# wangheda/youtube-8m

Measured on AMD Instinct MI355X. Metric: training videos/sec, higher is better.
Workload: dtype f32; 1 GPU; BASELINE configs[3]: LstmModel (2 x BasicLSTMCell(1024), dynamic_rnn over F=300) on raw uint8 [B,300,1152] frames + MoeModel head (2 mixtures, V=4716), fp32 training step (fwd+bwd+clip+Adam); per_gpu_batch=128, global_batch=128, frames=300, parallelism=dp1, params=113902808

## Files before the change

include/yt8m_hip.h:

```cpp
#ifndef YT8M_HIP_H
#define YT8M_HIP_H
#include <stdint.h>

#ifdef __cplusplus
extern "C" {
#endif

typedef void* yt8m_stream_t;

enum yt8m_status { YT8M_OK = 0, YT8M_E_BADARG = -1, YT8M_E_SHAPE = -2, YT8M_E_HIP = -3, YT8M_E_RCCL = -4 };
enum yt8m_label_dtype { YT8M_LABEL_U8 = 0, YT8M_LABEL_F32 = 1 };

int yt8m_abi_version(void);
const char* yt8m_last_error(void);
const char* yt8m_built_arch(void);

int yt8m_prof_enable(int on);
int yt8m_prof_reset(void);
int yt8m_prof_get(int family, int64_t* launches, double* total_ms);
int yt8m_prof_get_flops(int family, double* flops);
int yt8m_prof_get_bytes(int family, double* bytes);

int yt8m_probe_mfma_f32(int iters, int blocks, float* sink, yt8m_stream_t stream);
int yt8m_probe_mfma_bf16(int iters, int blocks, int random_operands, float* sink, yt8m_stream_t stream);
int yt8m_probe_copy_f32(const float* src, float* dst, int64_t n, yt8m_stream_t stream);
int yt8m_probe_placement(int* out, int blocks, int spin_ticks, yt8m_stream_t stream);
int yt8m_stream_create_cu_mask(const uint32_t* mask, int words, yt8m_stream_t* stream);
int yt8m_stream_destroy(yt8m_stream_t stream);

int yt8m_gemm_f32(int transA, int transB, int64_t M, int64_t N, int64_t K,
                  const float* A, int64_t lda, const float* B, int64_t ldb,
                  float* C, int64_t ldc, const float* bias, float beta, yt8m_stream_t stream);

int yt8m_gemm_f32_batched(int transA, int transB, int64_t M, int64_t N, int64_t K,
                          const float* A, int64_t lda, int64_t strideA, const float* B, int64_t ldb, int64_t strideB,
                          float* C, int64_t ldc, int64_t strideC, float beta, int64_t batch, yt8m_stream_t stream);

typedef struct yt8m_gemm_problem {
  int64_t M, N, K;
  const void* A; int64_t lda;
  const void* B; int64_t ldb;
  float* C; int64_t ldc;
  const float* bias;
  float beta;
} yt8m_gemm_problem;
int64_t yt8m_gemm_workspace_bytes(void);
int yt8m_gemm_f32_grouped(int transA, int transB, int nprob, const yt8m_gemm_problem* probs, void* workspace,
                          int64_t workspace_bytes, yt8m_stream_t stream);
int yt8m_gemm_bf16_nt_grouped(int nprob, const yt8m_gemm_problem* probs, void* workspace, int64_t workspace_bytes,
                              yt8m_stream_t stream);
int64_t yt8m_x3_image_bytes(int64_t rows, int64_t K);
int yt8m_x3_split(const float* src, int64_t R, int64_t C, int64_t ld, float scale, void* plain, void* trans, yt8m_stream_t stream);
int yt8m_gemm_x3_nt_grouped(int nprob, const yt8m_gemm_problem* probs, void* workspace, int64_t workspace_bytes,
                            yt8m_stream_t stream);
int yt8m_h2_split(const float* src, int64_t R, int64_t C, int64_t ld, float scale, const float* dscale, void* plain, void* trans,
                  float* colpart, yt8m_stream_t stream);
int yt8m_h2_absmax(const float* src, int64_t R, int64_t C, int64_t ld, void* word, yt8m_stream_t stream);
int yt8m_h2_degraded(uint64_t* counts, int reset, yt8m_stream_t stream);
int yt8m_h2_split_dropout(const float* src, int64_t R, int64_t C, float scale, const float* dscale, void* plain, void* trans,
                          float keep_prob, uint64_t seed, int64_t offset, yt8m_stream_t stream);
int yt8m_h2_split_rowmax(const float* src, int64_t R, int64_t C, int64_t ld, const void* rowmax, float* inv, void* plain,
                         yt8m_stream_t stream);
int yt8m_h2_split_ex(const float* src, int64_t R, int64_t C, int64_t ld, float scale, const void* dscale, const float* rowscale, void* plain,
                     void* trans, void* trans_scaled, float* colpart, float* colpart_scaled, yt8m_stream_t stream);
int yt8m_gemm_h1x2_nt_ex(int64_t M, int64_t N, int64_t K, const void* A1, int64_t ska, const void* B2, int64_t skb, float* C, int64_t ldc,
                         const float* bias, float alpha, const void* dsb, const float* rowscale, const float* colsum, float colsum_scale,
                         float beta, void* workspace, int64_t workspace_bytes, yt8m_stream_t stream);
int yt8m_h2_rowscales(const float* src, int64_t R, int64_t C, int64_t ld, float* S, float* inv, yt8m_stream_t stream);
int yt8m_h2_split_rows(const float* src, int64_t R, int64_t C, int64_t ld, const float* S, void* plain, yt8m_stream_t stream);
int yt8m_gemm_h2_nt_ex(int64_t M, int64_t N, int64_t K, const void* A2, int64_t ska, const void* B2, int64_t skb, float* C, int64_t ldc,
                       const float* bias, float alpha, const void* dsa, const void* dsb, const float* rowscale, float beta, void* workspace,
                       int64_t workspace_bytes, yt8m_stream_t stream);
int yt8m_timepool_max_f32(const float* y, int64_t F, int64_t B, int64_t N, int64_t ldy, float* out, int32_t* idx, int64_t ldo,
                          yt8m_stream_t stream);
int yt8m_timepool_shiftmax_f32(const float* z, int64_t F, int64_t B, int64_t ldz, int nfilt, const int32_t* fs, const int32_t* ncol, float* out,
                               int32_t* idx, int64_t ldo, yt8m_stream_t stream);
int yt8m_u8_cnn_pool_dw(const uint8_t* q, const float* r_tm, const int32_t* idx, const float* g, int64_t ldg, int64_t B, int64_t F, int64_t D,
                        int64_t N, int64_t fs, float* dW, float beta, yt8m_stream_t stream);
int yt8m_f32_cnn_pool_dw(const float* x, int64_t ldx, const int32_t* idx, const float* g, int64_t ldg, int64_t B, int64_t F, int64_t D,
                         int64_t N, int64_t fs, float* dW, int64_t lddw, float beta, yt8m_stream_t stream);
int yt8m_f32_cnn_pool_dx(const int32_t* idx, const float* g, int64_t ldg, int64_t B, int64_t F, int64_t D, int nfilt, const float* const* wt,
                         const int32_t* fs, const int32_t* ncol, float* dx, int64_t lddx, yt8m_stream_t stream);
int yt8m_u8_frames_image_f16(const uint8_t* q, const int32_t* num_frames, int64_t B, int64_t F, int64_t D, float eps, void* image,
                             float* x_tm, float* r_out, yt8m_stream_t stream);
int yt8m_u8_frames_image_t_f16(const uint8_t* q, const int32_t* num_frames, int64_t B, int64_t F, int64_t D, void* image_t,
                               yt8m_stream_t stream);
int yt8m_gemm_h2_nt_grouped(int nprob, const yt8m_gemm_problem* probs, const float* alphas, const float* const* dsa,
                            const float* const* dsb, void* workspace, int64_t workspace_bytes, yt8m_stream_t stream);
int yt8m_x3_set_combine(int mode);
int yt8m_x3_set_schedule(int mode);
#define YT8M_GEMM_ROLE_DW 0x100
#define YT8M_GEMM_ROLE_H2 0x200
int yt8m_gemm_x3_pays(int64_t M, int64_t N, int64_t K);
int64_t yt8m_gemm_auto_scratch_bytes(int transA, int transB, int nprob, const yt8m_gemm_problem* probs);
int yt8m_gemm_auto_grouped(int transA, int transB, int nprob, const yt8m_gemm_problem* probs, void* workspace,
                           int64_t workspace_bytes, void* image_scratch, int64_t image_scratch_bytes, uint64_t* used_x3,
                           yt8m_stream_t stream);
int yt8m_gemm_auto_grouped_ex(int transA, int transB, int nprob, const yt8m_gemm_problem* probs, const float* const* absmaxA,
                              const float* const* absmaxB, void* workspace, int64_t workspace_bytes, void* image_scratch,
                              int64_t image_scratch_bytes, uint64_t* used_x3, yt8m_stream_t stream);
int yt8m_gemm_x1x3_nt(int64_t M, int64_t N, int64_t K, const void* A1, const void* B3, float* C, int64_t ldc, const float* bias,
                      const float* rowscale, const float* colsum, float colsum_scale, void* workspace, int64_t workspace_bytes,
                      yt8m_stream_t stream);
int yt8m_gemm_x1x3_nt_ex(int64_t M, int64_t N, int64_t K, const void* A1, int64_t ska, const void* B3, int64_t skb, float* C,
                         int64_t ldc, const float* bias, float alpha, const float* rowscale, const float* colsum,
                         float colsum_scale, float beta, void* workspace, int64_t workspace_bytes, yt8m_stream_t stream);
int yt8m_bf16_image(const float* src, int64_t R, int64_t C, int64_t ld, float scale, void* plain, void* trans, yt8m_stream_t stream);
int yt8m_gemm_b1_nt_grouped(int nprob, const yt8m_gemm_problem* probs, void* workspace, int64_t workspace_bytes, yt8m_stream_t stream);
int yt8m_gemm_b1_nt_grouped_bf16c(int nprob, const yt8m_gemm_problem* probs, unsigned c_bf16_mask, void* workspace, int64_t workspace_bytes,
                                  yt8m_stream_t stream);
int yt8m_moe_mix_fwd_bf16z(const void* Zg, const void* Ze, float* p, int64_t B, int64_t V, int M, yt8m_stream_t stream);
int yt8m_moe_mix_bwd_bf16_images_z16(const void* Zg, const void* Ze, const float* dp, const void* labels, int label_dtype, int64_t B,
                                     int64_t V, int M, float eps, float dscale, const float* upstream_dev, void* dZg_img, int64_t g_kb,
                                     void* dZg_t_img, int64_t gt_kb, void* dZe_img, int64_t e_kb, void* dZe_t_img, int64_t et_kb,
                                     float* be_part, yt8m_stream_t stream);
int yt8m_bf16_image_colsum(const float* src, int64_t R, int64_t C, int64_t ld, float scale, const float* rowscale, void* plain,
                           void* trans, void* trans_scaled, float* colpart, float* colpart_scaled, yt8m_stream_t stream);
int yt8m_gemm_b1_nt_ex(int64_t M, int64_t N, int64_t K, const void* A1, int64_t ska, const void* B1, int64_t skb, float* C, int64_t ldc,
                       const float* bias, float alpha, const float* rowscale, const float* colsum, float colsum_scale, float beta,
                       void* workspace, int64_t workspace_bytes, yt8m_stream_t stream);
int yt8m_x3_split_ex(const float* src, int64_t R, int64_t C, int64_t ld, float scale, const float* rowscale, void* plain,
                     void* trans, void* trans_scaled, yt8m_stream_t stream);
int yt8m_x3_split_colsum(const float* src, int64_t R, int64_t C, int64_t ld, float scale, const float* rowscale, void* plain,
                         void* trans, void* trans_scaled, float* colpart, float* colpart_scaled, yt8m_stream_t stream);
int yt8m_cast_f32_bf16(const float* src, int64_t rows, int64_t cols, int64_t ld, void* dst, int64_t dst_ld, int transpose,
                       yt8m_stream_t stream);
int yt8m_cast_f32_bf16_dual(const float* src, int64_t rows, int64_t cols, int64_t ld, void* dst_plain, int64_t plain_ld,
                            void* dst_trans, int64_t trans_ld, yt8m_stream_t stream);

int yt8m_l2norm_fwd_f32(const float* x, float* y, int64_t rows, int64_t cols, float eps, yt8m_stream_t stream);
int yt8m_l2norm_bwd_f32(const float* x, const float* dy, float* dx, int64_t rows, int64_t cols, float eps,
                        yt8m_stream_t stream);
int yt8m_dequant_l2norm_u8(const uint8_t* q, const int32_t* num_frames, float* x,
                           int64_t B, int64_t F, int64_t D, float eps, yt8m_stream_t stream);
int yt8m_dequant_mean_l2norm_u8(const uint8_t* q, const int32_t* num_frames, float* x,
                                int64_t B, int64_t F, int64_t D, float eps, yt8m_stream_t stream);
int yt8m_resolution_mean_u8(const uint8_t* q, const int32_t* num_frames, float* y, int32_t* num_frames_out, int64_t B, int64_t F,
                            int64_t D, int64_t resolution, int l2norm, float eps, yt8m_stream_t stream);
int yt8m_resolution_mean_f32(const float* x, const int32_t* num_frames, float* y, int32_t* num_frames_out, int64_t B, int64_t F,
                             int64_t D, int64_t resolution, int l2norm, float eps, yt8m_stream_t stream);
int yt8m_frame_pyramid_u8(const uint8_t* q, const int32_t* num_frames, int64_t B, int64_t F, int64_t D, int levels, int nseg,
// ... 586 lines not shown
```

youtube-8m_amd/_lib.py:

```python
import ctypes
import os

_HERE = os.path.dirname(os.path.abspath(__file__))
LIB_PATH = os.environ.get("YT8M_LIB", os.path.join(_HERE, "libyt8m_hip.so"))

c_void_p, c_int, c_int64, c_float, c_double = ctypes.c_void_p, ctypes.c_int, ctypes.c_int64, ctypes.c_float, ctypes.c_double
P = c_void_p

class GemmProblem(ctypes.Structure):
    _fields_ = [("M", c_int64), ("N", c_int64), ("K", c_int64), ("A", c_void_p), ("lda", c_int64), ("B", c_void_p),
                ("ldb", c_int64), ("C", c_void_p), ("ldc", c_int64), ("bias", c_void_p), ("beta", c_float)]


STREAM_HOOK = ctypes.CFUNCTYPE(None, ctypes.c_void_p, ctypes.c_void_p)


class PersistBwdImages(ctypes.Structure):
    _fields_ = [("plain", ctypes.c_void_p), ("trans", ctypes.c_void_p), ("trans_scaled", ctypes.c_void_p), ("rowscale", ctypes.c_void_p),
                ("colpart", ctypes.c_void_p), ("colpart_scaled", ctypes.c_void_p)]


class LstmStackDesc(ctypes.Structure):
    _fields_ = [("B", c_int64), ("F", c_int64), ("D", c_int64), ("H", c_int64), ("L", ctypes.c_int32), ("input_u8", ctypes.c_int32),
                ("forget_bias", c_float), ("fwd_chunks", ctypes.c_int32), ("bwd_chunks", ctypes.c_int32), ("need_dx", ctypes.c_int32),
# ... 196 lines not shown
    "yt8m_lstm_persist_fwd_bf16": (c_int, [P, P, c_int64, P, P, P, P, c_int64, c_int64, c_int64, c_int64, c_float, P, c_int64, P]),
    "yt8m_lstm_persist_bwd_supported": (c_int, [c_int64, c_int64]),
    "yt8m_lstm_persist_bwd": (c_int, [P, P, c_int64, P, P, P, P, c_int, P, P, c_int64, c_int64, c_int64, c_int64, P, c_int64, P]),
    "yt8m_lstm_persist_bwd_bf16": (c_int, [P, P, c_int64, P, P, P, P, c_int, P, P, c_int64, c_int64, c_int64, c_int64, P, c_int64, P]),
    "yt8m_lstm_persist_fwd_h2": (c_int, [P, P, c_int64, P, P, P, P, c_int64, c_int64, c_int64, c_int64, c_float, P, P, c_int64, P]),
    "yt8m_lstm_persist_bwd_h2": (c_int, [P, P, c_int64, P, P, P, P, c_int, P, P, c_int64, c_int64, c_int64, c_int64, P, P, c_int64, P]),
    "yt8m_lstm_persist_bwd_on_f16_pipe": (c_int, [c_int64, c_int64]),
    "yt8m_lstm_persist_bwd_ex": (c_int, [P, P, c_int64, P, P, P, P, c_int, P, c_int64, c_int64, c_int64, c_int64, P, P, P, P, c_int64, P]),
    "yt8m_h2_split_rowmax": (c_int, [P, c_int64, c_int64, c_int64, P, P, P, P]),
    "yt8m_lstm_persist_bwd_images_rows": (c_int, [c_int64, c_int64]),
    "yt8m_lstm_persist_bwd_images": (c_int, [P, P, c_int64, P, P, P, P, c_int, P, c_int64, c_int64, c_int64, c_int64, P, c_int64, P, P]),
    "yt8m_lstm_packed_floats": (c_int64, [c_int64, c_int64]),
    "yt8m_lstm_pack": (c_int, [P, c_int64, c_int64, P, P, P]),
    "yt8m_lstm_steps_fwd": (c_int, [P, P, c_int64, P, P, P, P, P, c_int64, c_int64, c_int64, c_int64, c_float, P, c_int64, P]),
    "yt8m_lstm_steps_bwd": (c_int, [P, P, c_int64, P, P, P, P, P, c_int, P, c_int64, c_int64, c_int64, c_int64, P, c_int64, P]),
    "yt8m_lstm_layer_bwd": (c_int, [P, P, c_int64, P, P, P, P, P, P, P, c_int64, c_int64, c_int64, P, c_int64, P]),
    "yt8m_attn_softmax_fwd": (c_int, [P, P, P, c_int64, c_int64, c_int64, P]),
    "yt8m_attn_softmax_bwd": (c_int, [P, P, P, P, c_int64, c_int64, c_int64, P]),
    "yt8m_softmax_rows_fwd": (c_int, [P, P, P, c_int64, c_int64, c_int64, P]),
    "yt8m_softmax_rows_bwd": (c_int, [P, P, P, P, c_int64, c_int64, c_int64, P]),
    "yt8m_netvlad_supported": (c_int, [c_int64, c_int64, c_int64, c_int64]),
    "yt8m_netvlad_single_pass": (c_int, [c_int64, c_int64, c_int64, c_int64]),
    "yt8m_netvlad_set_single": (c_int, [c_int]),
    "yt8m_netvlad_workspace_bytes": (c_int64, [c_int64, c_int64, c_int64, c_int64]),
    "yt8m_netvlad_fwd_u8": (c_int, [P, P, P, P, c_int64, c_int64, c_int64, c_int64, c_int, c_float, P, P, P, P, c_int64, P]),
    "yt8m_netvlad_bwd_u8": (c_int, [P, P, P, P, P, c_int64, c_int64, c_int64, c_int64, c_int, c_float, P, c_float, P, c_float,
                                    P, c_int64, P]),
    "yt8m_vlad_finish_fwd": (c_int, [P, P, P, P, P, c_int64, c_int64, c_int64, c_int64, c_float, P]),
    "yt8m_vlad_finish_bwd": (c_int, [P, P, P, P, P, P, P, c_float, c_int64, c_int64, c_int64, c_float, P]),
    "yt8m_vlad_finish_q_supported": (c_int, [c_int64]),
    "yt8m_vlad_finish_q_fwd": (c_int, [P, P, P, P, P, P, c_int64, c_int64, c_int64, c_int64, c_float, P]),
    "yt8m_vlad_finish_q_bwd": (c_int, [P, P, P, P, P, P, P, P, c_float, c_int64, c_int64, c_int64, c_float, P]),
    "yt8m_crc32c": (ctypes.c_uint32, [P, c_int64]),
    "yt8m_crc32c_masked": (ctypes.c_uint32, [P, c_int64]),
    "yt8m_prefetch_open": (c_int, [ctypes.POINTER(ctypes.c_char_p), c_int, c_int, ctypes.POINTER(ctypes.c_char_p),
                                   ctypes.POINTER(ctypes.c_int32), c_int, c_int64, c_int64, c_int64, c_int, c_int, c_int,
                                   ctypes.POINTER(c_void_p)]),
    "yt8m_prefetch_acquire": (c_int, [P, ctypes.POINTER(c_void_p), ctypes.POINTER(c_void_p), ctypes.POINTER(c_void_p),
                                      ctypes.POINTER(c_void_p), ctypes.POINTER(c_int64), ctypes.POINTER(c_int64),
                                      ctypes.POINTER(c_int)]),
    "yt8m_prefetch_close": (c_int, [P]),
    "yt8m_tfrecord_write_predictions": (c_int, [ctypes.c_char_p, c_int64, P, c_int64, P, P, c_int64, ctypes.c_char_p]),
    "yt8m_tfrecord_open": (c_int, [ctypes.c_char_p, c_int, ctypes.POINTER(c_void_p)]),
    "yt8m_tfrecord_close": (c_int, [P]),
    "yt8m_tfrecord_read_frame_batch": (c_int, [P, ctypes.POINTER(ctypes.c_char_p), ctypes.POINTER(ctypes.c_int32), c_int, c_int64,
                                               c_int64, c_int64, P, P, P, P, c_int64, ctypes.POINTER(c_int64)]),
    "yt8m_tfrecord_read_video_batch": (c_int, [P, ctypes.POINTER(ctypes.c_char_p), ctypes.POINTER(ctypes.c_int32), c_int, c_int64,
                                               c_int64, P, P, P, c_int64, ctypes.POINTER(c_int64)]),
    "yt8m_comm_unique_id": (c_int, [P]),
    "yt8m_comm_init": (c_int, [c_int, c_int, P, ctypes.POINTER(c_void_p)]),
    "yt8m_comm_size": (c_int, [P, ctypes.POINTER(c_int), ctypes.POINTER(c_int)]),
    "yt8m_comm_allreduce_f32": (c_int, [P, P, c_int64, c_int, P]),
    "yt8m_comm_allreduce_mean": (c_int, [P, P, c_int64, P]),
    "yt8m_comm_allreduce_rsag_f32": (c_int, [P, P, c_int64, c_int, c_int, P]),
    "yt8m_comm_broadcast_f32": (c_int, [P, P, c_int64, c_int, P]),
    "yt8m_comm_destroy": (c_int, [P]),
    "yt8m_u8_proj_supported": (c_int, [c_int64]),
    "yt8m_u8_frames_to_bf16_tm": (c_int, [P, P, c_int64, c_int64, c_int64, c_float, c_int, P, c_int64, P, P, P]),
    "yt8m_split3_bf16_t": (c_int, [P, c_int64, c_int64, c_int64, c_float, P, c_int64, P]),
    "yt8m_rowscale_bias_f32": (c_int, [P, c_int64, c_int64, c_int64, P, P, c_float, P, P]),
    "yt8m_sample_frames_f32": (c_int, [P, P, c_int64, c_int64, c_int64, c_int64, c_int, ctypes.c_uint64, P, P, P]),
    "yt8m_sample_frames_u8": (c_int, [P, P, c_int64, c_int64, c_int64, c_int64, c_int, ctypes.c_uint64, P, P, P]),
    "yt8m_frame_pool_fwd": (c_int, [P, c_int64, c_int64, c_int64, c_int, P, P]),
    "yt8m_frame_pool_bwd": (c_int, [P, P, P, c_int64, c_int64, c_int64, c_int, P, P]),
    "yt8m_batchnorm_fwd": (c_int, [P, c_int64, c_int64, P, P, P, P, c_int, c_float, c_float, P, P, P, P]),
    "yt8m_batchnorm_workspace_bytes": (c_int64, [c_int64]),
    "yt8m_batchnorm_bwd": (c_int, [P, P, c_int64, c_int64, P, P, P, c_int, P, P, c_float, P, c_float, P, c_int64, P]),
    "yt8m_wimg_register": (c_int, [P, c_int64, c_int64, c_int64, c_int, c_int, c_float, P]),
    "yt8m_wimg_unregister": (c_int64, [P, P]),
    "yt8m_wimg_lookup": (c_void_p, [P, c_int64, c_int64, c_int64, c_int, c_int, c_float]),
    "yt8m_wimg_count": (c_int64, []),
    "yt8m_wimg_watch": (c_int, [P, P, c_int]),
    "yt8m_wimg_note_demand": (c_int, [P, c_int64, c_int64, c_int64, c_int, c_int, c_float]),
    "yt8m_wimg_demands": (c_int64, [ctypes.POINTER(WimgDemand), c_int64]),
    "yt8m_wimg_demand_generation": (c_int64, [P, P]),
    "yt8m_wimg_jobs_layout": (c_int64, [ctypes.POINTER(WimgJob), c_int64]),
    "yt8m_adam_tiles": (c_int, [P, P, P, P, P, c_int64, c_int64, c_int64, P, c_float, P, c_float, c_float, c_float, c_float, c_float,
                                c_int, P]),
    "yt8m_adam_multi_ex": (c_int, [P, P, P, P, P, c_int64, P, c_float, P, c_float, c_float, c_float, c_float, c_float, P, P]),
    "yt8m_optimizer_ranges": (c_int, [ctypes.POINTER(OptRanges), P]),
    "yt8m_lstm_stack_set_early_optimizer": (c_int, [ctypes.POINTER(OptRanges)]),
    "yt8m_h2_split": (c_int, [P, c_int64, c_int64, c_int64, c_float, P, P, P, P, P]),
    "yt8m_h2_absmax": (c_int, [P, c_int64, c_int64, c_int64, P, P]),
    "yt8m_h2_degraded": (c_int, [ctypes.POINTER(ctypes.c_uint64), c_int, P]),
    "yt8m_clip_by_norm_f32": (c_int, [P, P, c_int64, c_float, P, P]),
    "yt8m_gru_persist_supported": (c_int, [c_int64, c_int64]),
    "yt8m_gru_persist_workspace_bytes": (c_int64, [c_int64, c_int64, c_int64]),
    "yt8m_gru_persist_fwd": (c_int, [P, P, P, c_int64, P, c_int64, P, P, P, P, c_int64, c_int64, c_int64, c_int64, P, c_int64, P]),
    "yt8m_h2_split_dropout": (c_int, [P, c_int64, c_int64, c_float, P, P, P, c_float, ctypes.c_uint64, c_int64, P]),
    "yt8m_h2_split_ex": (c_int, [P, c_int64, c_int64, c_int64, c_float, P, P, P, P, P, P, P, P]),
    "yt8m_gemm_h1x2_nt_ex": (c_int, [c_int64, c_int64, c_int64, P, c_int64, P, c_int64, P, c_int64, P, c_float, P, P, P, c_float, c_float, P,
                                     c_int64, P]),
    "yt8m_h2_rowscales": (c_int, [P, c_int64, c_int64, c_int64, P, P, P]),
    "yt8m_h2_split_rows": (c_int, [P, c_int64, c_int64, c_int64, P, P, P]),
    "yt8m_gemm_h2_nt_ex": (c_int, [c_int64, c_int64, c_int64, P, c_int64, P, c_int64, P, c_int64, P, c_float, P, P, P, c_float, P, c_int64, P]),
    "yt8m_timepool_max_f32": (c_int, [P, c_int64, c_int64, c_int64, c_int64, P, P, c_int64, P]),
    "yt8m_timepool_shiftmax_f32": (c_int, [P, c_int64, c_int64, c_int64, c_int, ctypes.POINTER(ctypes.c_int32), ctypes.POINTER(ctypes.c_int32), P, P,
                                           c_int64, P]),
    "yt8m_u8_cnn_pool_dw": (c_int, [P, P, P, P, c_int64, c_int64, c_int64, c_int64, c_int64, c_int64, P, c_float, P]),
    "yt8m_f32_cnn_pool_dw": (c_int, [P, c_int64, P, P, c_int64, c_int64, c_int64, c_int64, c_int64, c_int64, P, c_int64, c_float, P]),
    "yt8m_f32_cnn_pool_dx": (c_int, [P, P, c_int64, c_int64, c_int64, c_int64, c_int, PP, ctypes.POINTER(ctypes.c_int32),
                                     ctypes.POINTER(ctypes.c_int32), P, c_int64, P]),
    "yt8m_u8_frames_image_f16": (c_int, [P, P, c_int64, c_int64, c_int64, c_float, P, P, P, P]),
    "yt8m_u8_frames_image_t_f16": (c_int, [P, P, c_int64, c_int64, c_int64, P, P]),
    "yt8m_gemm_h2_nt_grouped": (c_int, [c_int, ctypes.POINTER(GemmProblem), ctypes.POINTER(c_float), PP, PP, P, c_int64, P]),
    "yt8m_topk_rows": (c_int, [P, c_int64, c_int64, c_int, P, P, P]),
    "yt8m_perr_rows": (c_int, [P, P, c_int64, c_int64, P, P]),
    "yt8m_reverse_sequence_u8": (c_int, [P, P, P, c_int64, c_int64, c_int64, P]),
    "yt8m_reverse_sequence_f32_tm": (c_int, [P, c_int64, P, P, c_int64, c_int64, c_int64, c_int64, c_int64, P]),
    "yt8m_lstm_stack_use_streams": (c_int, [c_int, ctypes.POINTER(c_int)]),
    "yt8m_half_segments_u8": (c_int, [P, P, P, P, c_int64, c_int64, c_int64, P]),
    "yt8m_half_segments_f32": (c_int, [P, P, P, P, c_int64, c_int64, c_int64, P]),
    "yt8m_half_segment_means_u8": (c_int, [P, P, P, c_int64, c_int64, c_int64, c_int, c_float, P]),
    "yt8m_dequant_noise_u8": (c_int, [P, P, P, c_int64, c_int64, c_int64, c_float, ctypes.c_uint64, P]),
    "yt8m_frame_subset_draw": (c_int, [P, c_int64, c_int64, c_int64, ctypes.c_uint64, P]),
    "yt8m_frame_subset_gather_u8": (c_int, [P, P, P, P, P, c_int64, c_int64, c_int64, c_int64, c_int64, P]),
    "yt8m_frame_subset_gather_f32": (c_int, [P, P, P, P, P, c_int64, c_int64, c_int64, c_int64, c_int64, P]),
    "yt8m_resolution_mean_u8": (c_int, [P, P, P, P, c_int64, c_int64, c_int64, c_int64, c_int, c_float, P]),
    "yt8m_resolution_mean_f32": (c_int, [P, P, P, P, c_int64, c_int64, c_int64, c_int64, c_int, c_float, P]),
    "yt8m_multiscale_workspace_bytes": (c_int64, [c_int64]),
    "yt8m_colmoments_f32": (c_int, [P, c_int64, c_int64, c_int64, P, P, c_int, c_float, c_float, P, P, P, c_int64, P]),
    "yt8m_bn_relu_pool2_tm_fwd": (c_int, [P, c_int64, c_int64, c_int64, c_int64, P, P, P, P, P, c_int64, P, c_int64, P]),
    "yt8m_bn_relu_pool2_tm_bwd": (c_int, [P, c_int64, c_int64, c_int64, c_int64, P, P, P, P, c_int, P, c_int64, P, c_int64, P, c_int64, P,
                                          c_float, P, c_float, P, c_int64, P]),
    "yt8m_timepool_max_pool2_f32_fwd": (c_int, [P, c_int64, c_int64, c_int64, c_int64, P, P, c_int64, P, c_int64, P]),
    "yt8m_timepool_max_pool2_f32_bwd": (c_int, [P, c_int64, c_int64, c_int64, c_int64, P, P, c_int64, P, c_int64, P, c_int64, P]),
    "yt8m_ens_max_gates": (c_int, []),
    "yt8m_ens_combine_fwd": (c_int, [P, P, P, c_int, P, P, c_int64, c_int64, c_int64, c_int, P]),
    "yt8m_ens_combine_bwd_workspace_bytes": (c_int64, [c_int64, c_int64, c_int64, c_int]),
    "yt8m_ens_combine_bwd": (c_int, [P, P, P, c_int, P, P, P, P, P, P, c_int64, c_int64, c_int64, c_int64, c_int, P]),
    "yt8m_ens_moments": (c_int, [P, P, P, c_int64, c_int64, c_int64, P]),
    "yt8m_ens_tensor_max_methods": (c_int, []),
    "yt8m_ens_tensor_fwd": (c_int, [P, P, P, P, P, c_int64, c_int64, c_int64, P]),
    "yt8m_ens_tensor_bwd_workspace_bytes": (c_int64, [c_int64, c_int64, c_int64]),
    "yt8m_ens_tensor_bwd": (c_int, [P, P, P, P, P, P, P, P, P, c_int64, c_int64, c_int64, c_int64, P]),
    "yt8m_ens_mix_fwd": (c_int, [P, P, P, c_int64, c_int64, c_int64, P]),
    "yt8m_ens_mix_bwd": (c_int, [P, P, P, c_int64, c_int64, c_int64, P]),
    "yt8m_sigattn_supported": (c_int, [c_int64] * 5),
    "yt8m_sigattn_workspace_bytes": (c_int64, [c_int64] * 5),
    "yt8m_sigattn_fwd": (c_int, [P, c_int64, P, c_int64, P, P, P, P, P, P, P, c_int64] + [c_int64] * 5 + [P]),
    "yt8m_sigattn_bwd": (c_int, [P, c_int64, P, c_int64] + [P] * 8 + [c_int64, P, c_int64, P, P, P, c_int64] + [c_int64] * 5 + [P]),
    "yt8m_smattn_supported": (c_int, [c_int64] * 5),
    "yt8m_smattn_workspace_bytes": (c_int64, [c_int64] * 5),
    "yt8m_smattn_fwd": (c_int, [P, c_int64, P, c_int64] + [P] * 9 + [c_int64] + [c_int64] * 5 + [P]),
    "yt8m_smattn_bwd": (c_int, [P, c_int64, P, c_int64] + [P] * 8 + [c_int64, P, c_int64, P, P, P, P, c_int64] + [c_int64] * 5 + [P]),
    "yt8m_scale_mix_supported": (c_int, [c_int, c_int64, c_int64]),
    "yt8m_scale_mix_fwd": (c_int, [c_int, PP, PP, P, c_int64, c_int64, P]),
    "yt8m_scale_mix_bwd": (c_int, [c_int, PP, PP, P, P, PP, PP, c_int64, c_int64, P]),
    "yt8m_lstm_wide_supported": (c_int, [c_int64, c_int64]),
    "yt8m_lstm_wide_row_tile": (c_int, []),
    "yt8m_lstm_wide_workspace_bytes": (c_int64, [c_int64, c_int64]),
    "yt8m_lstm_wide_prepare": (c_int, [P, c_int64, c_int64, c_int64, P, c_int64, P]),
    "yt8m_lstm_wide_steps_fwd": (c_int, [P, P, c_int64, P, P, P, c_int64, c_int64, c_int64, c_int64, c_float, P]),
    "yt8m_distill_input_supported": (c_int, [c_int64, c_int64, c_int64]),
    "yt8m_distill_input_fwd": (c_int, [c_int, P, P, P, c_int64, c_int64, c_int64, P, P, P, P, c_int64, c_int64, c_int64, c_float, P]),
    "yt8m_distill_input_bwd": (c_int, [c_int, P, P, P, P, P, P, P, P, c_int64, c_int64, c_int64, P]),
    "yt8m_distill_blend_supported": (c_int, [c_int64, c_int64, c_int64]),
    "yt8m_distill_blend_fwd": (c_int, [P, P, c_int64, P, c_int64, c_int64, c_int64, c_float, P]),
    "yt8m_distill_blend_bwd": (c_int, [P, P, c_int64, c_int64, c_int64, c_float, P]),
    "yt8m_mix_link_supported": (c_int, [c_int64, c_int64]),
    "yt8m_mix_link_fwd": (c_int, [c_int, P, P, P, P, P, c_int64, c_int64, c_int64, c_float, c_float, P]),
    "yt8m_mix_link_bwd": (c_int, [c_int, P, P, P, P, P, P, c_int64, c_int64, c_int64, c_int64, c_float, P]),
    "yt8m_softmax_moe_supported": (c_int, [c_int64, c_int64]),
    "yt8m_softmax_moe_resident": (c_int, [c_int64, c_int64]),
    "yt8m_softmax_moe_fwd": (c_int, [P, P, P, P, P, c_int64, c_int64, c_int64, c_int64, P]),
    "yt8m_softmax_moe_bwd": (c_int, [P, P, P, P, c_int64, c_int64, P, P, c_int64, c_int64, c_int64, P]),
# ... 43 lines not shown
```

youtube-8m_amd/ops.py:

```python
import ctypes
import os

import torch

from . import _lib
from . import wimg as _wimg
from .flags import FLAGS, DEFINE_string
from .variables import get_default_graph

DEFINE_string("compute_dtype", "float32", "float32 (exact fp32 MFMA) or bfloat16 (bf16 MFMA operands, fp32 accumulate, fp32 "
              "master weights / gradients / optimiser) for the fully-connected and MoE-head GEMMs; the fused NetVLAD pooling "
              "uses single-f16 operands instead of the f16 hi+lo split.")

ACT = {"sigmoid": 0, "relu": 1, "relu6": 2, "tanh": 3, "elu": 4}
XENT_EPS = 10e-6


def _p(t):
    return ctypes.c_void_p(t.data_ptr()) if t is not None else None


def _stream():
    return ctypes.c_void_p(torch.cuda.current_stream().cuda_stream)

# ... 1902 lines not shown
        else:
            product([pg, pe], **kw)
            Wg.grad_done()
            We.grad_done()
    if be.grad is not None:
        colsum(bsrc, be.grad.view(-1), beta=be.grad_beta())
        be.grad_done()


def _moe_head_bwd_bf16_fused(ctx, x, Zg, Ze, Wg, We, be, V, M, dp=None, labels=None, ldt=0, dscale=1.0, up=None):
    L = _lib.lib()
    B = Zg.shape[0]
    dev = Zg.device
    if _b1_ok(B, Zg.shape[1], x.shape[1]) and _b1_ok(x.shape[1], Zg.shape[1], B):
        return _moe_head_bwd_bf16_images(ctx, x, Zg, Ze, Wg, We, be, V, M, dp, labels, ldt, dscale, up)
    Zgb, ZgT = _bf16_empty(B, Zg.shape[1], dev), _bf16_empty(Zg.shape[1], B, dev)
    Zeb, ZeT = _bf16_empty(B, Ze.shape[1], dev), _bf16_empty(Ze.shape[1], B, dev)
    part = torch.empty((L.yt8m_moe_mix_bwd_bf16_partial_rows(B), Ze.shape[1]), dtype=torch.float32, device=dev) \
        if be.grad is not None else None
    _lib.check(L.yt8m_moe_mix_bwd_bf16(_p(Zg), _p(Ze), _p(dp), _p(labels), ldt, B, V, M, XENT_EPS, float(dscale), _p(up),
                                       _p(Zgb), Zgb.stride(0), _p(ZgT), ZgT.stride(0), _p(Zeb), Zeb.stride(0), _p(ZeT),
                                       ZeT.stride(0), _p(part), _stream()))
    dx = None
    if ctx.needs_input_grad[0]:
        dx, = gemm_bf16_nt_grouped([dict(A=Zgb, B=cast_bf16(Wg.data))])
        gemm_bf16_nt_grouped([dict(A=Zeb, B=cast_bf16(We.data), out=dx, beta=1.0)])
    del Zgb, Zeb
    pg = pe = None
    if Wg.grad is not None and We.grad is not None:
        xT = cast_bf16(x, transpose=True)
        pg = dict(A=xT, B=ZgT, out=Wg.grad, beta=Wg.grad_beta())
        pe = dict(A=xT, B=ZeT, out=We.grad, beta=We.grad_beta())
    _moe_head_dw(gemm_bf16_nt_grouped, pg, pe, Wg, We, be, part)
    return dx


def _moe_head_bwd_bf16_images(ctx, x, Zg, Ze, Wg, We, be, V, M, dp, labels, ldt, dscale, up):
    L = _lib.lib()
    B, Ng, Ne = Zg.shape[0], Zg.shape[1], Ze.shape[1]
    dev = Zg.device
    Zgi, ZgTi, Zei, ZeTi = _image_empty(B, Ng, 1, dev), _image_empty(Ng, B, 1, dev), _image_empty(B, Ne, 1, dev), _image_empty(Ne, B, 1, dev)
    part = torch.empty((L.yt8m_moe_mix_bwd_bf16_partial_rows(B), Ne), dtype=torch.float32, device=dev) if be.grad is not None else None
    kb = lambda K: (K + 15) // 16
    mix = L.yt8m_moe_mix_bwd_bf16_images_z16 if Zg.dtype == torch.bfloat16 else L.yt8m_moe_mix_bwd_bf16_images
    _lib.check(mix(_p(Zg), _p(Ze), _p(dp), _p(labels), ldt, B, V, M, XENT_EPS, float(dscale), _p(up),
                   _p(Zgi.buf), kb(Ng), _p(ZgTi.buf), kb(B), _p(Zei.buf), kb(Ne), _p(ZeTi.buf), kb(B), _p(part), _stream()))
    kept = getattr(ctx, "images", None) or {}
    ctx.images = None
    dx = None
    if ctx.needs_input_grad[0]:
        dx, = gemm_b1_grouped([dict(A=Zgi, B=kept.get("Wg") or bf16_image(Wg.data))])
        gemm_b1_grouped([dict(A=Zei, B=kept.get("We") or bf16_image(We.data), out=dx, beta=1.0)])
    del Zgi, Zei
    pg = pe = None
    if Wg.grad is not None and We.grad is not None:
        xT = kept.get("xT") or bf16_image(x, transpose=True)
        pg = dict(A=xT, B=ZgTi, out=Wg.grad, beta=Wg.grad_beta())
        pe = dict(A=xT, B=ZeTi, out=We.grad, beta=We.grad_beta())
    _moe_head_dw(gemm_b1_grouped, pg, pe, Wg, We, be, part)
    return dx


def _fused_mix_bf16_ok(ctx, x, Zg, Ze, M):
    return (FUSED_MIX_BF16 and getattr(ctx, "bf16", False) and M == 2 and _bf16_ok(x) and Zg.shape[1] % 2 == 0
            and Ze.shape[1] % 2 == 0 and Zg.is_contiguous() and Ze.is_contiguous())


def _bf16_ok(x2):
    return x2.shape[0] % 2 == 0 and x2.shape[1] % 2 == 0 and x2.shape[0] >= BF16_MIN_ROWS


Z16_LOGITS = os.environ.get("YT8M_Z16_LOGITS", "0") != "0"
MOE_LOGITS_H2 = os.environ.get("YT8M_MOE_LOGITS_H2", "1") != "0"
MOE_LOGITS_H2_MIN_ROWS = int(os.environ.get("YT8M_MOE_LOGITS_H2_MIN_ROWS", "512"))
LINEAR_FWD_H2 = os.environ.get("YT8M_LINEAR_FWD_H2", "1") != "0"
LINEAR_H2_MIN_ROWS = int(os.environ.get("YT8M_LINEAR_H2_MIN_ROWS", "512"))
LINEAR_DX_H2 = os.environ.get("YT8M_LINEAR_DX_H2", "1") != "0"
LINEAR_H2_MIN_MNK = float(os.environ.get("YT8M_LINEAR_H2_MIN_MNK", "1e9"))
MOE_DX_H2 = os.environ.get("YT8M_MOE_DX_H2", "1") != "0"
MOE_DX_FROM = os.environ.get("YT8M_MOE_DX_FROM", "1") != "0"
MIX_BWD_ABSMAX = os.environ.get("YT8M_MIX_BWD_ABSMAX", "1") != "0"


def _z16_ok(x2, Wg, We, V, M, bf16, training):
    B, D = x2.shape
    Ng = Wg.data.shape[1]
    if not (Z16_LOGITS and bf16 and M == 2 and _bf16_ok(x2) and V % 4 == 0 and Ng == 3 * V and We.data.shape[1] == 2 * V):
        return False
    if not _b1_ok(B, Ng, D):
        return False
    if training and not (FUSED_MIX_BF16 and _b1_ok(D, Ng, B) and Wg.grad is not None and We.grad is not None):
        return False
    return True


def _moe_logits(x2, Wg, We, be, bf16, keep=None, z16=False, words=None):
    if bf16 and _bf16_ok(x2) and _b1_ok(x2.shape[0], Wg.data.shape[1], x2.shape[1]):
        odt = torch.bfloat16 if z16 else torch.float32
        if keep is not None and _b1_ok(x2.shape[1], Wg.data.shape[1], x2.shape[0]):
            xi, keep["xT"] = bf16_image(x2, both=True)
            keep["Wg"], WgT = bf16_image(Wg.data, both=True)
            keep["We"], WeT = bf16_image(We.data, both=True)
            return gemm_b1_grouped([dict(A=xi, B=WgT, out_dtype=odt), dict(A=xi, B=WeT, bias=be.data, out_dtype=odt)])
        xi = bf16_image(x2)
        return gemm_b1_grouped([dict(A=xi, B=bf16_image(Wg.data, transpose=True), out_dtype=odt),
                                dict(A=xi, B=bf16_image(We.data, transpose=True), bias=be.data, out_dtype=odt)])
    if bf16 and _bf16_ok(x2):
        xb = cast_bf16(x2)
        return gemm_bf16_nt_grouped([dict(A=xb, B=cast_bf16(Wg.data, transpose=True)),
                                     dict(A=xb, B=cast_bf16(We.data, transpose=True), bias=be.data)])
    h2 = MOE_LOGITS_H2 and x2.shape[0] >= MOE_LOGITS_H2_MIN_ROWS
    xmax = h2_absmax(x2).view(torch.float32) if (h2 and words is not None) else None
    if xmax is not None:
        words["x"] = xmax
    return gemm_grouped([dict(A=x2, B=Wg.data, absmaxA=xmax), dict(A=x2, B=We.data, bias=be.data, absmaxA=xmax)], role="h2" if h2 else None)


class _MoeHeadXent(torch.autograd.Function):

    @staticmethod
    def forward(ctx, x, token, Wg, We, be, labels, V, M, bf16):
        x2, Zg, Ze = _moe_head_fwd(ctx, x, Wg, We, be, V, M, bf16)
        B = x2.shape[0]
        lab, ldt = _labels_arg(labels)
        if tuple(lab.shape) != (B, V):
            raise ValueError("labels shape %s != predictions shape %s" % (tuple(lab.shape), (B, V)))
        L = _lib.lib()
        ws = torch.empty((L.yt8m_moe_mix_xent_workspace_bytes(B, V) + 3) // 4, dtype=torch.float32, device=x2.device)
        p = torch.empty((B, V), dtype=torch.float32, device=x2.device)
        loss = torch.empty((), dtype=torch.float32, device=x2.device)
        _lib.check(L.yt8m_moe_mix_xent_fwd(_p(Zg), _p(Ze), _p(lab), ldt, _p(p), _p(loss), B, V, M, XENT_EPS, _p(ws), _stream()))
        ctx.lab = (lab, ldt)
        ctx.mark_non_differentiable(p)
        ctx.set_materialize_grads(False)
        return p, loss

    @staticmethod
    def backward(ctx, dp_unused, dloss):
        (x,) = ctx.saved_tensors
        Zg, Ze = ctx.Z
        Wg, We, be = ctx.vars
        lab, ldt = ctx.lab
        V, M = ctx.VM
        ctx.Z = None
        if dloss is None:
            return (None,) * 9
        if _fused_mix_bf16_ok(ctx, x, Zg, Ze, M):
            dx = _moe_head_bwd_bf16_fused(ctx, x, Zg, Ze, Wg, We, be, V, M, labels=lab, ldt=ldt, dscale=1.0 / x.shape[0],
                                          up=_f32c(dloss.reshape(1)))
            return dx, None, None, None, None, None, None, None, None
        zmax = None
        if MIX_BWD_ABSMAX:
            zmax = torch.empty(2, dtype=torch.float32, device=Zg.device)
            _lib.check(_lib.lib().yt8m_moe_mix_xent_bwd_absmax(_p(Zg), _p(Ze), _p(lab), ldt, _p(_f32c(dloss.reshape(1))), x.shape[0], V, M,
                                                               XENT_EPS, 1.0, _p(zmax), _stream()))
        else:
            _lib.check(_lib.lib().yt8m_moe_mix_xent_bwd(_p(Zg), _p(Ze), _p(lab), ldt, _p(_f32c(dloss.reshape(1))), x.shape[0], V, M,
                                                        XENT_EPS, 1.0, _stream()))
        dx = _moe_head_param_grads(ctx, x, Zg, Ze, Wg, We, be, zmax=zmax, xmax=ctx.words.get("x"))
        return dx, None, None, None, None, None, None, None, None


def _moe_head_param_grads_bf16(ctx, x, Zg, Ze, Wg, We, be):
    dx = None
    need_dw = Wg.grad is not None and We.grad is not None
    dx_bf16 = ctx.needs_input_grad[0] and Zg.shape[1] % 2 == 0 and Ze.shape[1] % 2 == 0
    ZgT = ZeT = None
    if ctx.needs_input_grad[0]:
        if dx_bf16:
            Zgb, ZgT = cast_bf16_both(Zg) if need_dw else (cast_bf16(Zg), None)
            Zeb, ZeT = cast_bf16_both(Ze) if need_dw else (cast_bf16(Ze), None)
            dx, = gemm_bf16_nt_grouped([dict(A=Zgb, B=cast_bf16(Wg.data))])
            gemm_bf16_nt_grouped([dict(A=Zeb, B=cast_bf16(We.data), out=dx, beta=1.0)])
            del Zgb, Zeb
        else:
            dx = gemm(Zg, Wg.data, transB=True)
            gemm(Ze, We.data, out=dx, transB=True, beta=1.0)
    pg = pe = None
    if need_dw:
        xT = cast_bf16(x, transpose=True)
        pg = dict(A=xT, B=ZgT if ZgT is not None else cast_bf16(Zg, transpose=True), out=Wg.grad, beta=Wg.grad_beta())
        pe = dict(A=xT, B=ZeT if ZeT is not None else cast_bf16(Ze, transpose=True), out=We.grad, beta=We.grad_beta())
    _moe_head_dw(gemm_bf16_nt_grouped, pg, pe, Wg, We, be, Ze)
    return dx


_SIDE = {}
DEFER_HEAD_DW = os.environ.get("YT8M_DEFER_HEAD_DW", "0") != "0"


def side_stream(graph):
    if not DEFER_HEAD_DW or graph is None or not getattr(graph, "defer_head_dw", False) or graph.grad_ready_hook is not None:
        return None
# ... 280 lines not shown
```

Before: 8299 videos/s.

## Add small-row MoE head logits kernel splitting fp32 weights to f16 hi/lo on the fly

Adds a dedicated HIP kernel for the MoE gate and expert logits when the batch has at most 128 rows. It reads the fp32 weights directly, splits them into f16 hi+lo in registers, and runs three-term MFMA products against a pre-split activation image staged in LDS by a producer wave. Gate and expert tiles are covered by one launch with XCD-aware tile mapping. Weight scale factors come from a rotating absmax state kept across calls instead of a per-call weight split. This targets the cost of building weight images or going through the general grouped GEMM when M is small and the weight stream dominates. The cost is a lagged weight scale, with clamp and flush counters kept to detect when that scale goes out of range.

```diff
diff --git a/include/yt8m_hip.h b/include/yt8m_hip.h
--- a/include/yt8m_hip.h
+++ b/include/yt8m_hip.h
@@ -57,6 +57,11 @@
                   float* colpart, yt8m_stream_t stream);
 int yt8m_h2_absmax(const float* src, int64_t R, int64_t C, int64_t ld, void* word, yt8m_stream_t stream);
 int yt8m_h2_degraded(uint64_t* counts, int reset, yt8m_stream_t stream);
+int yt8m_moe_head_rows_supported(int64_t rows, int64_t K);
+int yt8m_moe_head_rows_state_words(void);
+int yt8m_moe_head_rows_logits(const void* ximg, const void* xword, int64_t rows, int64_t K, const float* Wg, int64_t Ng, const float* We,
+                              int64_t Ne, const float* be, float* Zg, float* Ze, void* state, int64_t call, yt8m_stream_t stream);
+int yt8m_moe_head_rows_counts(void* state, uint64_t* counts, int reset, yt8m_stream_t stream);
 int yt8m_h2_split_dropout(const float* src, int64_t R, int64_t C, float scale, const float* dscale, void* plain, void* trans,
                           float keep_prob, uint64_t seed, int64_t offset, yt8m_stream_t stream);
 int yt8m_h2_split_rowmax(const float* src, int64_t R, int64_t C, int64_t ld, const void* rowmax, float* inv, void* plain,
diff --git a/youtube-8m_amd/_lib.py b/youtube-8m_amd/_lib.py
--- a/youtube-8m_amd/_lib.py
+++ b/youtube-8m_amd/_lib.py
@@ -302,6 +302,10 @@
     "yt8m_lstm_stack_set_early_optimizer": (c_int, [ctypes.POINTER(OptRanges)]),
     "yt8m_h2_split": (c_int, [P, c_int64, c_int64, c_int64, c_float, P, P, P, P, P]),
     "yt8m_h2_absmax": (c_int, [P, c_int64, c_int64, c_int64, P, P]),
+    "yt8m_moe_head_rows_supported": (c_int, [c_int64, c_int64]),
+    "yt8m_moe_head_rows_state_words": (c_int, []),
+    "yt8m_moe_head_rows_logits": (c_int, [P, P, c_int64, c_int64, P, c_int64, P, c_int64, P, P, P, P, c_int64, P]),
+    "yt8m_moe_head_rows_counts": (c_int, [P, P, c_int, P]),
     "yt8m_h2_degraded": (c_int, [ctypes.POINTER(ctypes.c_uint64), c_int, P]),
     "yt8m_clip_by_norm_f32": (c_int, [P, P, c_int64, c_float, P, P]),
     "yt8m_gru_persist_supported": (c_int, [c_int64, c_int64]),
diff --git a/youtube-8m_amd/csrc/moe_head_rows.hip b/youtube-8m_amd/csrc/moe_head_rows.hip
--- /dev/null
+++ b/youtube-8m_amd/csrc/moe_head_rows.hip
@@ -0,0 +1,291 @@
+#include "common.h"
+#include "x3_image.h"
+
+namespace {
+
+typedef float f32x16 __attribute__((ext_vector_type(16)));
+typedef _Float16 f16x8 __attribute__((ext_vector_type(8)));
+typedef unsigned u32x4 __attribute__((ext_vector_type(4)));
+
+constexpr int TN = 96;
+constexpr int SK = 4;
+constexpr int ST_CLAMP = 6, ST_FLUSH = 7;
+constexpr int ST_WORDS = 8;
+
+struct LogitsArgs {
+  const u32x4* ximg;
+  const unsigned* xword;
+  const float* Wg;
+  const float* We;
+  const float* be;
+  float* Zg;
+  float* Ze;
+  unsigned* state;
+  int Ng, Ne, tiles_g, tiles, per_xcd;
+  int rows, K;
+  int cur, nxt, zero;
+};
+
+__device__ __forceinline__ f16x8 frag(const u32x4& v) { return __builtin_bit_cast(f16x8, v); }
+
+__device__ __forceinline__ void split8(const float (&w)[8], float sw, f16x8& hi, f16x8& lo, float& m, float& smin, float& chk) {
+  float t = 0.f;
+#pragma unroll
+  for (int j = 0; j < 8; ++j) {
+    float v = w[j] * sw;
+    m = fmaxf(m, fabsf(w[j]));
+    smin = fminf(smin, fabsf(v));
+    t += w[j];
+    v = fminf(fmaxf(v, -65504.f), 65504.f);
+    const _Float16 h = (_Float16)v;
+    hi[j] = h;
+    lo[j] = (_Float16)(v - (float)h);
+  }
+  chk = fmaf(0.f, t, chk);
+}
+
+template <int RG>
+__global__ __launch_bounds__(256) void moe_rows_logits_kernel(const LogitsArgs a) {
+  __shared__ u32x4 sX[2][4 * SK * 2 * 64];
+  __shared__ float sMax[3];
+  const int tid = threadIdx.x, lane = tid & 63;
+  const int w = __builtin_amdgcn_readfirstlane(tid >> 6);
+  const int bt = (int)(blockIdx.x & 7u) * a.per_xcd + (int)(blockIdx.x >> 3);
+  if (bt >= a.tiles) return;
+  const bool expert = bt >= a.tiles_g;
+  const int tile = bt - (expert ? a.tiles_g : 0);
+  const float* __restrict__ W = expert ? a.We : a.Wg;
+  float* __restrict__ Z = expert ? a.Ze : a.Zg;
+  const float* __restrict__ bias = expert ? a.be : nullptr;
+  const int N = expert ? a.Ne : a.Ng;
+  const int KB = a.K >> 4, NS = (KB + SK - 1) / SK;
+  if (bt == 0 && tid == 0) {
+    a.state[2 * a.zero] = 0u;
+    a.state[2 * a.zero + 1] = 0u;
+  }
+
+  if (w == 3) {
+    u32x4 xr[RG][2 * SK];
+    auto load_x = [&](int s) {
+#pragma unroll
+      for (int q = 0; q < RG; ++q) {
+#pragma unroll
+        for (int i = 0; i < 2 * SK; ++i) {
+          const int kb = s * SK + (i >> 1);
+          const u32x4 v = a.ximg[((int64_t)(q * KB + min(kb, KB - 1)) * 2 + (i & 1)) * 64 + lane];
+          xr[q][i] = kb < KB ? v : u32x4{0u, 0u, 0u, 0u};
+        }
+      }
+    };
+    auto write_x = [&](int buf) {
+#pragma unroll
+      for (int q = 0; q < RG; ++q) {
+#pragma unroll
+        for (int i = 0; i < 2 * SK; ++i) sX[buf][(q * 2 * SK + i) * 64 + lane] = xr[q][i];
+      }
+    };
+    load_x(0);
+    write_x(0);
+    if (NS > 1) load_x(1);
+    __syncthreads();
+    for (int s = 0; s < NS; ++s) {
+      if (s + 1 < NS) write_x((s + 1) & 1);
+      if (s + 2 < NS) load_x(s + 2);
+      __syncthreads();
+    }
+    __syncthreads();
+    return;
+  }
+
+  const int r = lane & 31, hh = lane >> 5;
+  const int slot = r * 2 + (hh ^ ((r >> 3) & 1));
+  const int n = tile * TN + w * 32 + r;
+  const bool col_ok = n < N;
+  const unsigned boff = 4u * ((unsigned)(hh * 8) * (unsigned)N + (unsigned)(col_ok ? n : N - 1));
+  const float sw = yt8m_x3::pow2_scale_for(__uint_as_float(a.state[2 * a.cur + (expert ? 1 : 0)]), 14);
+  const unsigned rowb = 4u * (unsigned)N;
+  const __amdgpu_buffer_rsrc_t wrs = __builtin_amdgcn_make_buffer_rsrc(const_cast<float*>(W), 0, (int)((unsigned)a.K * rowb), 0x00020000);
+  float wb[3][SK][8];
+  auto load_w = [&](float (&dst)[SK][8], int s) {
+#pragma unroll
+    for (int i = 0; i < SK; ++i) {
+      const int kb = min(s * SK + i, KB - 1);
+#pragma unroll
+      for (int j = 0; j < 8; ++j)
+        dst[i][j] = __builtin_bit_cast(float, __builtin_amdgcn_raw_buffer_load_b32(wrs, (int)boff, (int)((unsigned)(kb * 16 + j) * rowb), 0));
+    }
+  };
+  f32x16 acc[RG];
+#pragma unroll
+  for (int q = 0; q < RG; ++q)
+#pragma unroll
+    for (int e = 0; e < 16; ++e) acc[q][e] = 0.f;
+  float wmax = 0.f, poison = 0.f;
+  unsigned n_clamp = 0u, n_flush = 0u;
+  auto compute = [&](const float (&src)[SK][8], int s) {
+    const u32x4* sx = sX[s & 1] + slot;
+    float m_st = 0.f, smin = 3.0e38f, chk = 0.f;
+    f16x8 bhi, blo, bhi_n, blo_n;
+    u32x4 af[RG][2], af_n[RG][2];
+    split8(src[0], sw, bhi, blo, m_st, smin, chk);
+#pragma unroll
+    for (int q = 0; q < RG; ++q) {
+      af[q][0] = sx[((q * SK) * 2) * 64];
+      af[q][1] = sx[((q * SK) * 2 + 1) * 64];
+    }
+#pragma unroll
+    for (int i = 0; i < SK; ++i) {
+      if (i + 1 < SK) {
+        split8(src[i + 1], sw, bhi_n, blo_n, m_st, smin, chk);
+#pragma unroll
+        for (int q = 0; q < RG; ++q) {
+          af_n[q][0] = sx[((q * SK + i + 1) * 2) * 64];
+          af_n[q][1] = sx[((q * SK + i + 1) * 2 + 1) * 64];
+        }
+      }
+#pragma unroll
+      for (int q = 0; q < RG; ++q) {
+        const f16x8 ahi = frag(af[q][0]), alo = frag(af[q][1]);
+        acc[q] = __builtin_amdgcn_mfma_f32_32x32x16_f16(alo, bhi, acc[q], 0, 0, 0);
+        acc[q] = __builtin_amdgcn_mfma_f32_32x32x16_f16(ahi, blo, acc[q], 0, 0, 0);
+        acc[q] = __builtin_amdgcn_mfma_f32_32x32x16_f16(ahi, bhi, acc[q], 0, 0, 0);
+      }
+      if (i + 1 < SK) {
+#pragma unroll
+        for (int g = 0; g < 3 * RG; ++g) {
+          __builtin_amdgcn_sched_group_barrier(0x008, 1, 0);
+          __builtin_amdgcn_sched_group_barrier(0x100, (2 * RG + 3 * RG - 1) / (3 * RG), 0);
+          __builtin_amdgcn_sched_group_barrier(0x002, (72 + 3 * RG - 1) / (3 * RG), 0);
+        }
+        bhi = bhi_n; blo = blo_n;
+#pragma unroll
+        for (int q = 0; q < RG; ++q) { af[q][0] = af_n[q][0]; af[q][1] = af_n[q][1]; }
+      }
+    }
+    wmax = fmaxf(wmax, m_st);
+    if (__any(m_st * sw > 65504.f || smin < 2.98023224e-8f || chk != chk)) {
+#pragma unroll
+      for (int i = 0; i < SK; ++i) {
+        if (s * SK + i < KB) {
+#pragma unroll
+          for (int j = 0; j < 8; ++j) {
+            const float x = src[i][j], v = fabsf(x * sw);
+            if (col_ok) {
+              n_clamp += (v > 65504.f && v < 3.0e38f) ? 1u : 0u;
+              n_flush += (v != 0.f && v < 2.98023224e-8f) ? 1u : 0u;
+            }
+            if (x != x) poison = x;
+          }
+        }
+      }
+    }
+  };
+  load_w(wb[0], 0);
+  load_w(wb[1], 1);
+  __syncthreads();
+  for (int s0 = 0;; s0 += 3) {
+    load_w(wb[2], s0 + 2);
+    __builtin_amdgcn_sched_barrier(0);
+    compute(wb[0], s0);
+    __syncthreads();
+    if (s0 + 1 >= NS) break;
+    load_w(wb[0], s0 + 3);
+    __builtin_amdgcn_sched_barrier(0);
+    compute(wb[1], s0 + 1);
+    __syncthreads();
+    if (s0 + 2 >= NS) break;
+    load_w(wb[1], s0 + 4);
+    __builtin_amdgcn_sched_barrier(0);
+    compute(wb[2], s0 + 2);
+    __syncthreads();
+    if (s0 + 3 >= NS) break;
+  }
+
+  const float inv = 1.0f / (sw * yt8m_x3::pow2_scale_for(__uint_as_float(a.xword[0]), 14));
+  poison += __shfl_xor(poison, 32, 64);
+  const float bn = ((bias && col_ok) ? bias[n] : 0.f) + poison;
+#pragma unroll
+  for (int q = 0; q < RG; ++q) {
+#pragma unroll
+    for (int reg = 0; reg < 16; ++reg) {
+      const int row = q * 32 + (reg & 3) + 8 * (reg >> 2) + 4 * hh;
+      if (col_ok && row < a.rows) Z[(int64_t)row * N + n] = acc[q][reg] * inv + bn;
+    }
+  }
+  wmax = wave_max(wmax);
+  if (lane == 0) sMax[w] = wmax;
+  if (__any((n_clamp | n_flush) != 0u)) {
+#pragma unroll
+    for (int o = 32; o > 0; o >>= 1) { n_clamp += __shfl_xor(n_clamp, o, 64); n_flush += __shfl_xor(n_flush, o, 64); }
+    if (lane == 0) {
+      if (n_clamp) atomicAdd(a.state + ST_CLAMP, n_clamp);
+      if (n_flush) atomicAdd(a.state + ST_FLUSH, n_flush);
+    }
+  }
+  __syncthreads();
+  if (tid == 0) {
+    const float m = fmaxf(fmaxf(sMax[0], sMax[1]), sMax[2]);
+    if (m > 0.f && m < 3.0e38f) atomicMax(a.state + 2 * a.nxt + (expert ? 1 : 0), __float_as_uint(m));
+  }
+}
+
+}
+
+using namespace yt8m;
+
+extern "C" int yt8m_moe_head_rows_state_words(void) { return ST_WORDS; }
+
+extern "C" int yt8m_moe_head_rows_supported(int64_t rows, int64_t K) {
+  return (rows >= 1 && rows <= 128 && K >= 16 && (K % 16) == 0 && K < (1LL << 20)) ? 1 : 0;
+}
+
+extern "C" int yt8m_moe_head_rows_logits(const void* ximg, const void* xword, int64_t rows, int64_t K, const float* Wg, int64_t Ng,
+                                         const float* We, int64_t Ne, const float* be, float* Zg, float* Ze, void* state, int64_t call,
+                                         yt8m_stream_t stream) {
+  YT8M_REQUIRE(rows >= 0 && K >= 0 && Ng >= 0 && Ne >= 0 && call >= 0, YT8M_E_SHAPE, "negative dimension");
+  if (rows == 0 || Ng + Ne == 0) return YT8M_OK;
+  YT8M_REQUIRE(yt8m_moe_head_rows_supported(rows, K), YT8M_E_SHAPE, "needs 1 <= rows <= 128, K % 16 == 0, 16 <= K < 2^20");
+  YT8M_REQUIRE(Ng >= 1 && Ne >= 1 && Ng < (1LL << 24) && Ne < (1LL << 24), YT8M_E_SHAPE, "1 <= Ng, Ne < 2^24");
+  YT8M_REQUIRE((K + 8) * (Ng > Ne ? Ng : Ne) < (1LL << 30), YT8M_E_SHAPE, "a weight tensor must stay below 2^30 elements");
+  YT8M_REQUIRE(ximg && xword && Wg && We && Zg && Ze && state, YT8M_E_BADARG, "null operand");
+  YT8M_REQUIRE((reinterpret_cast<uintptr_t>(ximg) & 15) == 0 && (reinterpret_cast<uintptr_t>(state) & 3) == 0, YT8M_E_BADARG,
+               "the image must be 16-byte aligned");
+  hipStream_t s = as_stream(stream);
+  unsigned* st = static_cast<unsigned*>(state);
+  if (call == 0) {
+    YT8M_HIP_CHECK(hipMemsetAsync(st, 0, ST_WORDS * sizeof(unsigned), s));
+    int rc = yt8m_h2_absmax(Wg, K, Ng, Ng, st, stream);
+    if (rc == YT8M_OK) rc = yt8m_h2_absmax(We, K, Ne, Ne, st + 1, stream);
+    if (rc != YT8M_OK) return rc;
+  }
+  LogitsArgs a;
+  a.ximg = static_cast<const u32x4*>(ximg);
+  a.xword = static_cast<const unsigned*>(xword);
+  a.Wg = Wg; a.We = We; a.be = be; a.Zg = Zg; a.Ze = Ze; a.state = st;
+  a.Ng = (int)Ng; a.Ne = (int)Ne; a.tiles_g = (int)cdiv(Ng, TN);
+  a.tiles = a.tiles_g + (int)cdiv(Ne, TN);
+  a.per_xcd = (a.tiles + 7) / 8;
+  a.rows = (int)rows; a.K = (int)K;
+  a.cur = (int)(call % 3); a.nxt = (int)((call + 1) % 3); a.zero = (int)((call + 2) % 3);
+  const double N = (double)(Ng + Ne);
+  ProfScope prof(F_GEMM_H2, s, 2.0 * (double)rows * (double)K * N, 4.0 * (double)K * N + 4.0 * (double)rows * N + 4.0 * (double)rows * (double)K);
+  const dim3 grid((unsigned)(8 * a.per_xcd)), block(256);
+  switch ((rows + 31) / 32) {
+    case 1: hipLaunchKernelGGL(moe_rows_logits_kernel<1>, grid, block, 0, s, a); break;
+    case 2: hipLaunchKernelGGL(moe_rows_logits_kernel<2>, grid, block, 0, s, a); break;
+    case 3: hipLaunchKernelGGL(moe_rows_logits_kernel<3>, grid, block, 0, s, a); break;
+    default: hipLaunchKernelGGL(moe_rows_logits_kernel<4>, grid, block, 0, s, a); break;
+  }
+  return launch_status("moe_rows_logits_kernel");
+}
+
+extern "C" int yt8m_moe_head_rows_counts(void* state, uint64_t* counts, int reset, yt8m_stream_t stream) {
+  YT8M_REQUIRE(state && counts, YT8M_E_BADARG, "null operand");
+  unsigned host[2] = {0u, 0u};
+  YT8M_HIP_CHECK(hipStreamSynchronize(as_stream(stream)));
+  YT8M_HIP_CHECK(hipMemcpy(host, static_cast<unsigned*>(state) + ST_CLAMP, sizeof(host), hipMemcpyDeviceToHost));
+  counts[0] = host[0];
+  counts[1] = host[1];
+  if (reset) YT8M_HIP_CHECK(hipMemset(static_cast<unsigned*>(state) + ST_CLAMP, 0, sizeof(host)));
+  return YT8M_OK;
+}
diff --git a/youtube-8m_amd/ops.py b/youtube-8m_amd/ops.py
--- a/youtube-8m_amd/ops.py
+++ b/youtube-8m_amd/ops.py
@@ -2008,6 +2008,45 @@
 MIX_BWD_ABSMAX = os.environ.get("YT8M_MIX_BWD_ABSMAX", "1") != "0"
 
 
+MOE_HEAD_ROWS = os.environ.get("YT8M_MOE_HEAD_ROWS", "1") != "0"
+
+
+def _moe_head_rows_ok(x2, Wg, We):
+    rows, K = x2.shape
+    N = Wg.data.shape[1] + We.data.shape[1]
+    return bool(MOE_HEAD_ROWS and rows <= 128 and rows * N * K >= LINEAR_H2_MIN_MNK and Wg.data.is_contiguous() and We.data.is_contiguous()
+                and Wg.data.shape[0] == K and We.data.shape[0] == K and _lib.lib().yt8m_moe_head_rows_supported(rows, K))
+
+
+def _moe_head_rows_state(Wg, We, device):
+    st = getattr(Wg, "_head_rows_state", None)
+    if st is None or st["We"] is not We or st["words"].device != device:
+        st = {"We": We, "words": torch.zeros(_lib.lib().yt8m_moe_head_rows_state_words(), dtype=torch.int32, device=device), "calls": 0}
+        Wg._head_rows_state = st
+    return st
+
+
+def moe_head_rows_logits(x, Wg, We, be, state, call):
+    _dev(x, Wg, We, be, state)
+    x = _f32c(x)
+    rows, K = x.shape
+    xword = h2_absmax(x)
+    xi = image_buffer(rows, K, 2, x.device)
+    L = _lib.lib()
+    _lib.check(L.yt8m_h2_split(_p(x), rows, K, K, 1.0, _p(xword), _p(xi), None, None, _stream()))
+    Zg = torch.empty((rows, Wg.shape[1]), dtype=torch.float32, device=x.device)
+    Ze = torch.empty((rows, We.shape[1]), dtype=torch.float32, device=x.device)
+    _lib.check(L.yt8m_moe_head_rows_logits(_p(xi), _p(xword), rows, K, _p(Wg), Wg.shape[1], _p(We), We.shape[1], _p(be), _p(Zg), _p(Ze),
+                                           _p(state), int(call), _stream()))
+    return Zg, Ze, xword
+
+
+def moe_head_rows_counts(state, reset=False):
+    counts = (ctypes.c_uint64 * 2)()
+    _lib.check(_lib.lib().yt8m_moe_head_rows_counts(_p(state), counts, 1 if reset else 0, _stream()))
+    return int(counts[0]), int(counts[1])
+
+
 def _z16_ok(x2, Wg, We, V, M, bf16, training):
     B, D = x2.shape
     Ng = Wg.data.shape[1]
@@ -2035,6 +2074,13 @@
         xb = cast_bf16(x2)
         return gemm_bf16_nt_grouped([dict(A=xb, B=cast_bf16(Wg.data, transpose=True)),
                                      dict(A=xb, B=cast_bf16(We.data, transpose=True), bias=be.data)])
+    if _moe_head_rows_ok(x2, Wg, We):
+        st = _moe_head_rows_state(Wg, We, x2.device)
+        Zg, Ze, xword = moe_head_rows_logits(x2, Wg.data, We.data, be.data, st["words"], st["calls"])
+        st["calls"] += 1
+        if words is not None:
+            words["x"] = xword.view(torch.float32)
+        return Zg, Ze
     h2 = MOE_LOGITS_H2 and x2.shape[0] >= MOE_LOGITS_H2_MIN_ROWS
     xmax = h2_absmax(x2).view(torch.float32) if (h2 and words is not None) else None
     if xmax is not None:
```

Result: no change. 8343 videos/s, median of 6 (+0.5%).
